# BillyXYB/TransEditor

Hardware: AMD Instinct MI355X
Metric: 256x256 images/sec/GPU, G+D fwd+bwd, batch 16; 1/2/4/8-GPU scaling (higher is better)
Workload: dtype f32

## Files before the change

include/te_hip.h:

```cpp
#ifndef TE_HIP_H
#define TE_HIP_H

#include <stdint.h>

#ifdef __cplusplus
extern "C" {
#endif

#define TE_ABI_VERSION 3

#define TE_ERR_NULL -1
#define TE_ERR_SHAPE -2
#define TE_ERR_UNSUPPORTED -3
#define TE_ERR_WORKSPACE -4

typedef void* te_stream_t;

int te_version(void);
const char* te_last_error_string(void);
const char* te_arch(void);

int te_bias_act_f32(float* out, const float* x, const float* b, const float* ref, int act, int grad,
                    float alpha, float scale, int64_t size_x, int64_t step_b, int64_t size_b,
                    te_stream_t stream);
// ... 20 lines not shown
                     int minor, int kh, int kw, int up_x, int up_y, int down_x, int down_y, int pad_x0,
                     int pad_x1, int pad_y0, int pad_y1, te_stream_t stream);
int te_upfirdn2d_f64(double* out, const double* x, const double* k, int64_t major, int in_h, int in_w,
                     int minor, int kh, int kw, int up_x, int up_y, int down_x, int down_y, int pad_x0,
                     int pad_x1, int pad_y0, int pad_y1, te_stream_t stream);


#define TE_CONV_3X3 0
#define TE_CONV_T2 1
#define TE_CONV_S2 2
#define TE_CONV_1X1 3
#define TE_CONV_3X3W 4
#define TE_CONV_3X3W6 5

#define TE_CONV_S2S6 6

#define TE_CONV_T2S6 7

#define TE_CONV_1X1S6 8

#define TE_PACK_FWD 0
#define TE_PACK_DGRAD 1
#define TE_PACK_SWAP 2
#define TE_PACK_WFWD 3
#define TE_PACK_WDGRAD 4
#define TE_PACK_W6FWD 5
#define TE_PACK_W6DGRAD 6
#define TE_PACK_S6FWD 7
#define TE_PACK_S6SWAP 8
#define TE_PACK_T6FWD 9
#define TE_PACK_T6SWAP 10
#define TE_PACK_P6FWD 11
#define TE_PACK_P6DGRAD 12

int64_t te_conv_packed_numel(int kind_pack, int Co, int Ci, int ksize);
int te_conv_pack_weights_f32(float* wp, const float* w, float wscale, int kind_pack, int Co, int Ci,
                             int ksize, te_stream_t stream);
int te_conv_pack_weights2_f32(float* wp_a, int kind_a, float* wp_b, int kind_b, const float* w, float wscale, int Co, int Ci,
                              int ksize, te_stream_t stream);

int te_conv_pack_weights_multi_f32(int n, float* const* wp, const float* const* w, const float* wscale, const int* kind_pack,
                                   const int* Co, const int* Ci, const int* ksize, te_stream_t stream);

int te_conv_f32(float* out, const float* in, const float* wp, const float* isc, const float* osc,
                const float* bias, int act, int kind, int B, int K, int M, int H, int W,
                te_stream_t stream);
int te_conv_splitk_count(int kind, int B, int K, int M, int H, int W);
int te_conv_wino_supported(int B, int K, int M, int H, int W);
int te_conv_wino6_supported(int B, int K, int M, int H, int W);
int te_conv_s2s6_supported(int B, int K, int M, int H, int W);
int te_conv_t2s6_supported(int B, int K, int M, int H, int W);
int te_conv_p1s6_supported(int B, int K, int M, int H, int W);
int te_conv_wino6_form(int form);
int te_conv_s2s6_form(int form);
int te_conv_t2s6_form(int form);
int64_t te_conv_t2s6_ws_floats(int B, int K, int H);
int te_conv_ws_f32(float* out, float* ws, const float* in, const float* wp, const float* isc, const float* osc,
                   const float* bias, int act, int kind, int B, int K, int M, int H, int W, te_stream_t stream);
int te_conv_res_f32(float* out, float* ws, const float* in, const float* wp, const float* isc, const float* osc,
                    const float* bias, const float* res, const float* mask_ref, float mask_gain, int act, int kind, int B,
                    int K, int M, int H, int W, te_stream_t stream);

int te_wgrad_slab_count(int kind, int B, int Co, int Ci, int H, int W);
int te_wgrad_pair_form(int kind, int Co, int Ci, int H, int W);
int te_wgrad_split_supported(int kind, int Co, int Ci, int H, int W);
int te_wgrad_split_bf16(int on);
int te_wgrad_t2_wide(int on);
enum { TE_WG6_FP32 = 0, TE_WG6_3X3 = 1, TE_WG6_3X3_PAIR = 2, TE_WG6_T2_WIDE = 3, TE_WG6_T2 = 4, TE_WG6_T2_MASKED = 5, TE_WG6_1X1 = 6 };
int te_wgrad6_form(int kind, int B, int Co, int Ci, int H, int W, int NB);
int te_wgrad_f32(float* slabs, const float* g, const float* x, int kind, int B, int Co, int Ci, int H,
                 int W, int S, te_stream_t stream);
int te_wgrad_group_plan(int kind, int B, int Co, int Ci, int H, int W, int* NB, int* S);
int te_wgrad_group_f32(float* slabs, const float* g, const float* x, int kind, int B, int Co, int Ci, int H, int W, int S, int NB,
                       te_stream_t stream);

int64_t te_wgrad_reduce_ws_floats(int B, int S, int Co, int Ci, int taps, int want_w, int want_isc, int want_osc);
int te_wgrad_reduce_f32(float* gw, float* gisc, float* gosc, float* ws, const float* slabs, const float* w,
                        float wscale, const float* isc, const float* osc, int B, int S, int Co, int Ci,
                        int taps, te_stream_t stream);

int te_rgb_supported(int M, int K, int HW);
int te_rgb_fwd_f32(float* out, const float* x, const float* w, const float* isc, const float* bias, float wscale, int B,
                   int K, int HW, te_stream_t stream);
int te_rgb_dgrad_f32(float* gx, const float* g, const float* w, const float* isc, float wscale, int B, int K, int HW,
                     te_stream_t stream);
int te_rgb_expand_f32(float* out, const float* x3, const float* w, const float* bias, int act, float wscale, int B, int K,
                      int HW, te_stream_t stream);
int te_rgb_wgrad_slab_count(int B, int K, int HW);
int te_rgb_wgrad_f32(float* slabs, const float* g, const float* x, int B, int K, int HW, int S, te_stream_t stream);
int te_rgb_wgrad_sum_f32(float* slabs, const float* g, const float* x, int B, int K, int HW, int S, te_stream_t stream);

int te_attn_fwd_f32(float* o, float* sim, const float* q, const float* k, const float* v, float scale,
                    int N, int G, int M, int L, int D, te_stream_t stream);
int te_attn_bwd_f32(float* gq, float* gk, float* gv, const float* go, const float* gsim_or_null,
                    const float* q, const float* k, const float* v, const float* sim, float scale, int N,
                    int G, int M, int L, int D, te_stream_t stream);

int te_blur_actgrad_tiles(int in_h, int in_w, int kh, int kw, int pad_x0, int pad_x1, int pad_y0, int pad_y1);
int te_blur_actgrad_f32(float* gx, float* partial, const float* g, const float* ref, const float* k, int64_t major, int in_h,
                        int in_w, int kh, int kw, int pad_x0, int pad_x1, int pad_y0, int pad_y1, float alpha, float scale,
                        te_stream_t stream);
int te_blur_gradact_f32(float* gx, float* partial, const float* g, const float* ref, const float* k, int64_t major, int in_h,
                        int in_w, int kh, int kw, int pad_x0, int pad_x1, int pad_y0, int pad_y1, float alpha, float scale,
                        te_stream_t stream);

int te_small_gemm_f32(float* c, float* pre, const float* a, const float* b, const float* bias, const float* residual,
// ... 90 lines not shown
```

transeditor_amd/_lib.py:

```python
import ctypes as C
import os

import torch

_HERE = os.path.dirname(os.path.abspath(__file__))
LIB_PATH = os.path.join(_HERE, 'libte_hip.so')
_lib = None

CONV_3X3, CONV_T2, CONV_S2, CONV_1X1, CONV_3X3W, CONV_3X3W6, CONV_S2S6, CONV_T2S6, CONV_1X1S6 = 0, 1, 2, 3, 4, 5, 6, 7, 8
(PACK_FWD, PACK_DGRAD, PACK_SWAP, PACK_WFWD, PACK_WDGRAD, PACK_W6FWD, PACK_W6DGRAD, PACK_S6FWD, PACK_S6SWAP, PACK_T6FWD,
 PACK_T6SWAP, PACK_P6FWD, PACK_P6DGRAD) = range(13)

_P, _I, _L, _F = C.c_void_p, C.c_int, C.c_int64, C.c_float
_SIGNATURES = {
    'te_version': (C.c_int, []),
    'te_last_error_string': (C.c_char_p, []),
    'te_arch': (C.c_char_p, []),
    'te_bias_act_f32': (C.c_int, [_P, _P, _P, _P, _I, _I, _F, _F, _L, _L, _L, _P]),
    'te_bias_act_f16': (C.c_int, [_P, _P, _P, _P, _I, _I, _F, _F, _L, _L, _L, _P]),
    'te_bias_act_f64': (C.c_int, [_P, _P, _P, _P, _I, _I, _F, _F, _L, _L, _L, _P]),
    'te_bias_act_bwd_ws_floats': (C.c_int64, [_L, _L, _L]),
    'te_bias_act_bwd_f32': (C.c_int, [_P, _P, _P, _P, _P, _F, _F, _L, _L, _L, _P]),
    'te_bias_act_bwd_rgb_supported': (C.c_int, [_L, _L, _L]),
    'te_bias_act_bwd_rgb_f32': (C.c_int, [_P, _P, _P, _P, _P, _P, _P, _P, _F, _F, _F, _L, _L, _L, _P]),
    'te_upfirdn2d_f32': (C.c_int, [_P, _P, _P, _L, _I, _I, _I, _I, _I, _I, _I, _I, _I, _I, _I, _I, _I,
                                   _P, _L, _I, _F, _F, _P]),
    'te_upfirdn2d_f16': (C.c_int, [_P, _P, _P, _L, _I, _I, _I, _I, _I, _I, _I, _I, _I, _I, _I, _I, _I, _P]),
    'te_upfirdn2d_f64': (C.c_int, [_P, _P, _P, _L, _I, _I, _I, _I, _I, _I, _I, _I, _I, _I, _I, _I, _I, _P]),
    'te_conv_packed_numel': (C.c_int64, [_I, _I, _I, _I]),
    'te_conv_pack_weights_f32': (C.c_int, [_P, _P, _F, _I, _I, _I, _I, _P]),
    'te_conv_pack_weights2_f32': (C.c_int, [_P, _I, _P, _I, _P, _F, _I, _I, _I, _P]),
    'te_conv_pack_weights_multi_f32': (C.c_int, [_I, _P, _P, _P, _P, _P, _P, _P, _P]),
    'te_conv_f32': (C.c_int, [_P, _P, _P, _P, _P, _P, _I, _I, _I, _I, _I, _I, _I, _P]),
    'te_conv_splitk_count': (C.c_int, [_I, _I, _I, _I, _I, _I]),
    'te_conv_wino_supported': (C.c_int, [_I, _I, _I, _I, _I]),
    'te_conv_wino6_supported': (C.c_int, [_I, _I, _I, _I, _I]),
    'te_conv_wino6_form': (C.c_int, [_I]),
    'te_conv_s2s6_form': (C.c_int, [_I]),
    'te_conv_t2s6_form': (C.c_int, [_I]),
    'te_conv_t2s6_ws_floats': (C.c_int64, [_I, _I, _I]),
    'te_conv_s2s6_supported': (C.c_int, [_I, _I, _I, _I, _I]),
    'te_conv_t2s6_supported': (C.c_int, [_I, _I, _I, _I, _I]),
    'te_conv_p1s6_supported': (C.c_int, [_I, _I, _I, _I, _I]),
    'te_conv_ws_f32': (C.c_int, [_P, _P, _P, _P, _P, _P, _P, _I, _I, _I, _I, _I, _I, _I, _P]),
    'te_conv_res_f32': (C.c_int, [_P, _P, _P, _P, _P, _P, _P, _P, _P, _F, _I, _I, _I, _I, _I, _I, _I, _P]),
    'te_wgrad_slab_count': (C.c_int, [_I, _I, _I, _I, _I, _I]),
    'te_wgrad_pair_form': (C.c_int, [_I, _I, _I, _I, _I]),
    'te_wgrad_split_supported': (C.c_int, [_I, _I, _I, _I, _I]),
    'te_wgrad_split_bf16': (C.c_int, [_I]),
    'te_wgrad_t2_wide': (C.c_int, [_I]),
    'te_wgrad6_form': (C.c_int, [_I, _I, _I, _I, _I, _I, _I]),
    'te_wgrad_f32': (C.c_int, [_P, _P, _P, _I, _I, _I, _I, _I, _I, _I, _P]),
    'te_wgrad_group_plan': (C.c_int, [_I, _I, _I, _I, _I, _I, _P, _P]),
    'te_wgrad_group_f32': (C.c_int, [_P, _P, _P, _I, _I, _I, _I, _I, _I, _I, _I, _P]),
    'te_wgrad_reduce_ws_floats': (C.c_int64, [_I, _I, _I, _I, _I, _I, _I, _I]),
    'te_wgrad_reduce_f32': (C.c_int, [_P, _P, _P, _P, _P, _P, _F, _P, _P, _I, _I, _I, _I, _I, _P]),
    'te_rgb_supported': (C.c_int, [_I, _I, _I]),
    'te_rgb_fwd_f32': (C.c_int, [_P, _P, _P, _P, _P, _F, _I, _I, _I, _P]),
    'te_rgb_dgrad_f32': (C.c_int, [_P, _P, _P, _P, _F, _I, _I, _I, _P]),
    'te_rgb_wgrad_sum_f32': (C.c_int, [_P, _P, _P, _I, _I, _I, _I, _P]),
    'te_rgb_expand_f32': (C.c_int, [_P, _P, _P, _P, _I, _F, _I, _I, _I, _P]),
    'te_rgb_wgrad_slab_count': (C.c_int, [_I, _I, _I]),
    'te_rgb_wgrad_f32': (C.c_int, [_P, _P, _P, _I, _I, _I, _I, _P]),
    'te_blur_actgrad_tiles': (C.c_int, [_I] * 8),
    'te_blur_actgrad_f32': (C.c_int, [_P, _P, _P, _P, _P, _L, _I, _I, _I, _I, _I, _I, _I, _I, _F, _F, _P]),
    'te_blur_gradact_f32': (C.c_int, [_P, _P, _P, _P, _P, _L, _I, _I, _I, _I, _I, _I, _I, _I, _F, _F, _P]),
    'te_small_gemm_f32': (C.c_int, [_P, _P, _P, _P, _P, _P, _P, _F, _I, _I, _I, _L, _L, _L, _L, _F, _F, _I, _P]),
    'te_small_gemm_batched_f32': (C.c_int, [_P, _P, _P, _P, _I, _L, _L, _L, _L, _P, _P, _I, _I, _I, _L, _L, _L, _L, _L, _L,
                                             _F, _F, _I, _P]),
    'te_layer_norm_supported': (C.c_int, [_L, _I]),
    'te_layer_norm_fwd_f32': (C.c_int, [_P, _P, _P, _L, _I, _F, _P]),
    'te_layer_norm_bwd_f32': (C.c_int, [_P, _P, _P, _P, _L, _I, _P]),
    'te_pixel_norm_supported': (C.c_int, [_L, _I, _I]),
    'te_pixel_norm_fwd_f32': (C.c_int, [_P, _P, _P, _L, _I, _I, _F, _P]),
    'te_pixel_norm_bwd_f32': (C.c_int, [_P, _P, _P, _P, _L, _I, _I, _P]),
    'te_demod_fwd_f32': (C.c_int, [_P, _P, _P, _P, _F, _F, _I, _I, _I, _I, _P]),
    'te_demod_bwd_f32': (C.c_int, [_P, _P, _P, _P, _P, _P, _P, _F, _I, _I, _I, _I, _I, _P]),
    'te_attn_fwd_f32': (C.c_int, [_P, _P, _P, _P, _P, _F, _I, _I, _I, _I, _I, _P]),
    'te_attn_bwd_f32': (C.c_int, [_P, _P, _P, _P, _P, _P, _P, _P, _P, _F, _I, _I, _I, _I, _I, _P]),
    'te_small_gemm_splitk_f32': (C.c_int, [_P, _P, _P, _I, _P, _P, _P, _P, _I, _I, _I, _L, _L, _L, _L, _F, _F, _I, _P]),
    'te_minibatch_stddev_fwd_f32': (C.c_int, [_P, _P, _I, _I, _I, _I, _F, _P]),
    'te_minibatch_stddev_bwd_f32': (C.c_int, [_P, _P, _P, _I, _I, _I, _I, _F, _P]),
    'te_mt_adam_f32': (C.c_int, [_P, _P, _I, _I, _I, C.c_double, C.c_double, C.c_double, C.c_double, _I, _P]),
    'te_mt_ema_f32': (C.c_int, [_P, _P, _I, _I, _I, C.c_double, _P]),
    'te_chan_scale_f32': (C.c_int, [_P, _P, _P, _L, _L, _P]),
    'te_chan_dot_f32': (C.c_int, [_P, _P, _P, _L, _L, _P]),
    'te_lpips_stem_fwd_f32': (C.c_int, [_P, _P, _P, _P, _I, _I, _I, _P]),
    'te_lpips_stem_dgrad_f32': (C.c_int, [_P, _P, _P, _P, _I, _I, _I, _P]),
    'te_maxpool2_fwd_f32': (C.c_int, [_P, _P, _L, _I, _I, _P]),
    'te_maxpool2_bwd_f32': (C.c_int, [_P, _P, _P, _L, _I, _I, _P]),
# ... 226 lines not shown
    Co, Ci, ks, _ = w.shape
    n = lib().te_conv_packed_numel(kind_pack, Co, Ci, ks)
    wp = torch.empty(n, device=w.device, dtype=w.dtype)
    _check(lib().te_conv_pack_weights_f32(_ptr(wp), _ptr(w), wscale, kind_pack, Co, Ci, ks, _stream()),
           'te_conv_pack_weights_f32')
    return wp


def conv_pack2(w, kind_a, kind_b, wscale=1.0):
    w = w.contiguous()
    Co, Ci, ks, _ = w.shape
    wa = torch.empty(lib().te_conv_packed_numel(kind_a, Co, Ci, ks), device=w.device, dtype=w.dtype)
    wb = torch.empty(lib().te_conv_packed_numel(kind_b, Co, Ci, ks), device=w.device, dtype=w.dtype)
    _check(lib().te_conv_pack_weights2_f32(_ptr(wa), kind_a, _ptr(wb), kind_b, _ptr(w), wscale, Co, Ci, ks, _stream()),
           'te_conv_pack_weights2_f32')
    return wa, wb


def conv_pack_multi(jobs):
    n = len(jobs)
    if not n:
        return
    for wp, w, _, _ in jobs:
        if not (w.is_contiguous() and wp.is_contiguous()):
            raise RuntimeError('te_hip: conv_pack_multi needs dense weights and buffers')
    arr = lambda ty, vals: (ty * n)(*vals)
    _check(lib().te_conv_pack_weights_multi_f32(
        n, arr(C.c_void_p, [_ptr(j[0]) for j in jobs]), arr(C.c_void_p, [_ptr(j[1]) for j in jobs]),
        arr(C.c_float, [float(j[3]) for j in jobs]), arr(C.c_int, [int(j[2]) for j in jobs]),
        arr(C.c_int, [j[1].shape[0] for j in jobs]), arr(C.c_int, [j[1].shape[1] for j in jobs]),
        arr(C.c_int, [j[1].shape[2] for j in jobs]), _stream()), 'te_conv_pack_weights_multi_f32')


def wino_ok(B, K, M, H, W):
    return bool(lib().te_conv_wino_supported(B, K, M, H, W))


def s2s6_ok(B, K, M, H, W):
    return bool(lib().te_conv_s2s6_supported(B, K, M, H, W))


def t2s6_ok(B, K, M, H, W):
    return bool(lib().te_conv_t2s6_supported(B, K, M, H, W))


def p1s6_ok(B, K, M, H, W):
    return bool(lib().te_conv_p1s6_supported(B, K, M, H, W))


def wino6_form(form=-1):
    return int(lib().te_conv_wino6_form(form))


def s2s6_form(form=-1):
    return int(lib().te_conv_s2s6_form(form))


def t2s6_form(form=-1):
    return int(lib().te_conv_t2s6_form(form))


def wino6_ok(B, K, M, H, W):
    return bool(lib().te_conv_wino6_supported(B, K, M, H, W))


def conv_out_shape(kind, B, M, H, W):
    if kind in (CONV_T2, CONV_T2S6):
        return (B, M, 2 * H + 1, 2 * W + 1)
    return (B, M, H, W)


def _aligned16(t):
    if t is None or t.data_ptr() % 16 == 0:
        return t
    return t.clone(memory_format=torch.contiguous_format)


def conv(x, wp, kind, M, H, W, isc=None, osc=None, bias=None, act=0, res=None, mask_ref=None, mask_gain=1.0):
    x = x.contiguous()
    if kind == CONV_1X1S6:
        x = _aligned16(x)
    res = _aligned16(res.contiguous()) if res is not None else None
    mask_ref = _aligned16(mask_ref.contiguous()) if mask_ref is not None else None
    B, K = x.shape[0], x.shape[1]
    out = torch.empty(conv_out_shape(kind, B, M, H, W), device=x.device, dtype=x.dtype)
    if res is not None and tuple(res.shape) != tuple(out.shape):
        raise RuntimeError(f'te_hip: residual {tuple(res.shape)} does not match the convolution output {tuple(out.shape)}')
    if mask_ref is not None and tuple(mask_ref.shape) != tuple(out.shape):
        raise RuntimeError(f'te_hip: mask reference {tuple(mask_ref.shape)} does not match the convolution output {tuple(out.shape)}')
    S = lib().te_conv_splitk_count(kind, B, K, M, H, W)
    if S < 1:
        raise RuntimeError(f'te_conv_splitk_count failed ({S})')
    ws = torch.empty((S,) + tuple(out.shape), device=x.device, dtype=x.dtype) if S > 1 else None
    if kind == CONV_T2S6:
        ws = torch.empty(B * K * H, device=x.device, dtype=x.dtype)
    _check(lib().te_conv_res_f32(_ptr(out), _ptr(ws), _ptr(x), _ptr(wp), _ptr(isc), _ptr(osc), _ptr(bias),
                                 _ptr(res), _ptr(mask_ref), mask_gain, act, kind, B, K, M, H, W,
                                 _stream()),
           'te_conv_res_f32')
    return out


def wgrad_slabs(g, x, kind, H, W, group=False):
    g, x = g.contiguous(), x.contiguous()
    B, Co, Ci = g.shape[0], g.shape[1], x.shape[1]
    taps = 1 if kind == CONV_1X1 else 9
# ... 636 lines not shown
```

transeditor_amd/csrc/split6_common.h:

```cpp
#pragma once
#include "conv_common.h"

typedef short bf16x8 __attribute__((ext_vector_type(8)));
typedef __bf16 bf16x2 __attribute__((ext_vector_type(2)));
typedef float f32x2 __attribute__((ext_vector_type(2)));
typedef float f32x2u __attribute__((ext_vector_type(2), aligned(4)));
typedef float f32x4u __attribute__((ext_vector_type(4), aligned(4)));
typedef unsigned u32x4 __attribute__((ext_vector_type(4)));

__device__ __forceinline__ void split6_barrier() { asm volatile("s_waitcnt lgkmcnt(0)\n\ts_barrier" ::: "memory"); }
__device__ __forceinline__ void split6_wait_vm() { asm volatile("s_waitcnt vmcnt(0)" ::: "memory"); }

__device__ __forceinline__ unsigned split6_piece(float te, float to) {
    const f32x2 t = {te, to};
    return __builtin_bit_cast(unsigned, __builtin_convertvector(t, bf16x2));
}
__device__ __forceinline__ unsigned split6_take(float te, float to, float& fe, float& fo) {
    const unsigned h = split6_piece(te, to);
    fe = __builtin_bit_cast(float, h << 16);
    fo = __builtin_bit_cast(float, h & 0xFFFF0000u);
    return h;
}
__device__ __forceinline__ void split6_pin(float& te, float& to, float& fe, float& fo) { asm volatile("" : "+v"(te), "+v"(to), "+v"(fe), "+v"(fo)); }
template <bool PIN_LOW = true>
__device__ __forceinline__ void split6_step4(int j, float ve, float vo, float& te, float& to, float& fe, float& fo, unsigned& h, unsigned& m, unsigned& l) {
    if (j == 0) {
        te = ve; to = vo;
        h = split6_take(te, to, fe, fo);
    } else if (j == 1) {
        te -= fe; to -= fo;
    } else if (j == 2) {
        m = split6_take(te, to, fe, fo);
    } else {
        te -= fe; to -= fo;
        l = split6_piece(te, to);
        if (PIN_LOW) asm volatile("" : "+v"(l));
    }
    split6_pin(te, to, fe, fo);
}
__device__ __forceinline__ void split6_step3(int j, float ve, float vo, float& te, float& to, float& fe, float& fo, unsigned& h, unsigned& m, unsigned& l) {
    if (j == 0) {
        te = ve; to = vo;
        h = split6_take(te, to, fe, fo);
    } else if (j == 1) {
        te -= fe; to -= fo;
        m = split6_take(te, to, fe, fo);
    } else {
        te -= fe; to -= fo;
        l = split6_piece(te, to);
    }
    split6_pin(te, to, fe, fo);
}

__device__ __forceinline__ void split6_product(int q, const bf16x8 (&a)[3], const bf16x8 (&b)[3], f32x16& big, f32x16& small) {
    constexpr int PA[6] = {1, 0, 2, 0, 1, 0}, PB[6] = {1, 2, 0, 1, 0, 0};
    f32x16& d = q < 5 ? small : big;
    d = __builtin_amdgcn_mfma_f32_32x32x16_bf16(a[PA[q]], b[PB[q]], d, 0, 0, 0);
}

__device__ __forceinline__ bool split6_tile(int ntiles, int nt8, int mblocks, int& tile, int& mb) {
    const int xcd = blockIdx.x & 7, jx = blockIdx.x >> 3;
    const int tq = jx / mblocks;
    mb = jx % mblocks;
    tile = nt8 ? (int)(((int64_t)xcd * ntiles) >> 3) + tq : tq * 8 + xcd;
    return tile < (nt8 ? (int)(((int64_t)(xcd + 1) * ntiles) >> 3) : ntiles);
}

template <auto KERNEL, class Args>
inline void split6_launch(dim3 grid, int threads, size_t lds, hipStream_t s, const Args& a) {
    static std::atomic<uint64_t> attr_done{0};
    te::allow_big_lds(attr_done, (const void*)KERNEL, 160 * 1024);
    KERNEL<<<grid, threads, lds, s>>>(a);
}
#define SPLIT6_LAUNCH_ISC(kernel, isc, blocks, threads, lds, s, a) \
    ((isc) ? split6_launch<kernel<true>>(blocks, threads, lds, s, a) : split6_launch<kernel<false>>(blocks, threads, lds, s, a))
```

transeditor_amd/csrc/wino6.hip:

```cpp
#include "split6_common.h"
#ifdef W6P_PROF
#define TE_PROF
#endif
#include "te_prof.h"

namespace {

constexpr int WT = 512, KC = 16, TW = 32, NP = TW / 2, BM = 64, TH = 8;
constexpr int U_CHUNKS = 36 * 2 * 64;

struct Wino6Args {
    float* out; const float* in; const u32x4* U; const float* isc; const float* osc; const float* bias; const float* res;
    const float* mref; float mgain; int act;
    int B, K, M, H, W, ntiles, mblocks, tiles_x, tiles_y, nt8;
    int lgpw;
};

constexpr int PH = 4, PR = PH + 2;
constexpr int TP_PLANE = PR * 2 * NP * 4;
constexpr int TP_DWORDS = 12 * TP_PLANE;
constexpr int GT = WT / 2;
constexpr int P_IN = (PR * NP * 8) / GT;
static_assert(PR * NP * 8 == P_IN * GT, "items must divide over the group");

PROF_BUFFER(w6p, 2048 * 8 * 8)
constexpr int SLOT0 = 21;

template <bool ISC>
__global__ __launch_bounds__(WT, 2) void wino6p_kernel(const Wino6Args p) {
    extern __shared__ __attribute__((aligned(16))) unsigned char smem_raw[];
    u32x4* ul = reinterpret_cast<u32x4*>(smem_raw);
    const int tid = threadIdx.x, lane = tid & 63, l31 = lane & 31, half = lane >> 5;
    const int wid = __builtin_amdgcn_readfirstlane(tid >> 6);
    const int grp = wid >> 2, wq = wid & 3, wm = wq >> 1, wrl = wq & 1, gt = tid & (GT - 1);
    unsigned* tl = reinterpret_cast<unsigned*>(smem_raw + U_CHUNKS * 16) + grp * TP_DWORDS;
    const u32x4* tl4 = reinterpret_cast<const u32x4*>(tl);
    int tile, mb;
    if (!split6_tile(p.ntiles, p.nt8, p.mblocks, tile, mb)) return;
    const int pwm = (1 << p.lgpw) - 1;
    const int tx = tile % p.tiles_x, ty = (tile / p.tiles_x) % p.tiles_y, b = (tile / (p.tiles_x * p.tiles_y)) << (4 - p.lgpw);
    const int x0 = tx * TW, y0 = ty * TH, yh = y0 + PH * grp;
    const float* inb = p.in + (size_t)b * p.K * p.H * p.W;
    const float* iscb = ISC ? p.isc + (size_t)b * p.K : nullptr;
    const bool has_left = x0 == 0, has_right = x0 + TW >= p.W, has_rowout = (yh == 0) || (yh + PH == p.H);

    f32x16 acc[4];
#pragma unroll
    for (int c = 0; c < 4; ++c)
#pragma unroll
        for (int r = 0; r < 16; ++r) acc[c][r] = 0.f;

    unsigned g_off[P_IN];
    int l_off[P_IN], e_flag[P_IN];
#pragma unroll
    for (int i = 0; i < P_IN; ++i) {
        const int e = gt + GT * i;
        const int jj = e & 15, q = (e >> 4) & 7, row = e >> 7;
        const int gy = yh - 1 + row;
        const int sj = jj >> p.lgpw, jl = jj & pwm;
        const bool left = x0 == 0 && jl == 0, right = x0 + TW >= p.W && jl == pwm, rowout = gy < 0 || gy >= p.H;
        e_flag[i] = (left ? 1 : 0) | (right ? 2 : 0) | (rowout ? 4 : 0);
        const int gyc = gy < 0 ? 0 : (gy >= p.H ? p.H - 1 : gy);
        g_off[i] = (unsigned)(sj * p.K * p.H * p.W + (2 * q * p.H + gyc) * p.W + x0 + 2 * jl - 1 + (left ? 1 : 0) - (right ? 1 : 0));
        l_off[i] = ((row * 2 + (q >> 2)) * NP + jj) * 4 + (q & 3);
    }
    const unsigned q2 = 2u * ((gt >> 4) & 7) + (unsigned)(((gt & 15) >> p.lgpw) * p.K);
    const size_t plane = (size_t)p.H * p.W;
// ... 159 lines not shown
    const size_t off0 = ((size_t)bo * p.M + mbase) * plane + (size_t)(y0 + 2 * wr + rr) * p.W + x0 + 2 * (jj & pwm);
    const float g_pos = p.act == 3 ? 1.4142135623730951f : 1.f;
    float scv[16], biv[16];
#pragma unroll
    for (int r = 0; r < 16; ++r) {
        const int m = mbase + (r & 3) + 8 * (r >> 2) + 4 * half;
        scv[r] = p.osc ? p.osc[(size_t)bo * p.M + m] : 1.f;
        biv[r] = p.bias ? p.bias[m] : 0.f;
    }
    f32x2 resv[16], mrefv[16];
    if (p.res) {
#pragma unroll
        for (int r = 0; r < 16; ++r)
            resv[r] = *reinterpret_cast<const f32x2*>(p.res + off0 + (size_t)((r & 3) + 8 * (r >> 2) + 4 * half) * plane);
    }
    if (p.mref) {
#pragma unroll
        for (int r = 0; r < 16; ++r)
            mrefv[r] = *reinterpret_cast<const f32x2*>(p.mref + off0 + (size_t)((r & 3) + 8 * (r >> 2) + 4 * half) * plane);
    }
#pragma unroll
    for (int r = 0; r < 16; ++r) {
        const int dm = (r & 3) + 8 * (r >> 2) + 4 * half;
        float v0 = acc[0][r] + acc[1][r] + acc[2][r];
        float v1 = acc[1][r] - acc[2][r] - acc[3][r];
        const float sc = scv[r], bi = biv[r];
        v0 = v0 * sc + bi;
        v1 = v1 * sc + bi;
        if (p.act >= 3) {
            v0 = (v0 > 0.f ? v0 : v0 * 0.2f) * g_pos;
            v1 = (v1 > 0.f ? v1 : v1 * 0.2f) * g_pos;
        }
        const size_t o = off0 + (size_t)dm * plane;
        if (p.res) { v0 += resv[r][0]; v1 += resv[r][1]; }
        if (p.mref) {
            v0 *= mrefv[r][0] > 0.f ? p.mgain : 0.2f * p.mgain;
            v1 *= mrefv[r][1] > 0.f ? p.mgain : 0.2f * p.mgain;
        }
        f32x2 v; v[0] = v0; v[1] = v1;
        *reinterpret_cast<f32x2*>(p.out + o) = v;
    }
}


template <bool ISC>
__global__ __launch_bounds__(WT, 2) void wino6q_kernel(const Wino6Args p) {
    extern __shared__ __attribute__((aligned(16))) unsigned char smem_raw[];
    u32x4* ul = reinterpret_cast<u32x4*>(smem_raw);
    const int tid = threadIdx.x, lane = tid & 63, l31 = lane & 31, half = lane >> 5;
    const int wid = __builtin_amdgcn_readfirstlane(tid >> 6);
    const int grp = wid >> 2, wq = wid & 3, wm = wq >> 1, wrl = wq & 1, gt = tid & (GT - 1);
    unsigned* tl = reinterpret_cast<unsigned*>(smem_raw + U_CHUNKS * 16) + grp * TP_DWORDS;
    const u32x4* tl4 = reinterpret_cast<const u32x4*>(tl);
    int tile, mbq;
    if (!split6_tile(p.ntiles, p.nt8, p.mblocks, tile, mbq)) return;
    const int tx = tile % p.tiles_x, ty = (tile / p.tiles_x) % p.tiles_y, b = tile / (p.tiles_x * p.tiles_y);
    const int x0 = tx * TW, y0 = ty * TH, yh = y0 + PH * grp;
    const float* inb = p.in + (size_t)b * p.K * p.H * p.W;
    const float* iscb = ISC ? p.isc + (size_t)b * p.K : nullptr;
    const bool has_left = x0 == 0, has_right = x0 + TW == p.W, has_rowout = (yh == 0) || (yh + PH == p.H);

    f32x16 acc[2][4];
#pragma unroll
    for (int m = 0; m < 2; ++m)
#pragma unroll
        for (int c = 0; c < 4; ++c)
#pragma unroll
            for (int r = 0; r < 16; ++r) acc[m][c][r] = 0.f;

    unsigned g_off[P_IN];
    int l_off[P_IN], e_flag[P_IN];
#pragma unroll
    for (int i = 0; i < P_IN; ++i) {
        const int e = gt + GT * i;
        const int jj = e & 15, q = (e >> 4) & 7, row = e >> 7;
        const int gy = yh - 1 + row;
        const bool left = x0 == 0 && jj == 0, right = x0 + TW == p.W && jj == NP - 1, rowout = gy < 0 || gy >= p.H;
        e_flag[i] = (left ? 1 : 0) | (right ? 2 : 0) | (rowout ? 4 : 0);
        const int gyc = gy < 0 ? 0 : (gy >= p.H ? p.H - 1 : gy);
        g_off[i] = (unsigned)((2 * q * p.H + gyc) * p.W + x0 + 2 * jj - 1 + (left ? 1 : 0) - (right ? 1 : 0));
        l_off[i] = ((row * 2 + (q >> 2)) * NP + jj) * 4 + (q & 3);
    }
    const unsigned q2 = 2u * ((gt >> 4) & 7);
    const size_t plane = (size_t)p.H * p.W;
    const int MT = p.M >> 5;
    f32x4 rin[P_IN][2];
    f32x2 rsc = {1.f, 1.f};
    const int nstage = p.K / KC, nimg = 2 * nstage;
    auto fetch_scales = [&](int s) {
        if (ISC) rsc = *reinterpret_cast<const f32x2u*>(iscb + s * KC + q2);
    };
    auto fetch_item = [&](int i, int s) {
#pragma unroll
        for (int h2 = 0; h2 < 2; ++h2)
            rin[i][h2] = *reinterpret_cast<const f32x4u*>(inb + ((size_t)s * KC + h2) * plane + g_off[i]);
    };
    auto issue_u = [&](int uh, int j) {
        const u32x4* us = p.U + (size_t)(j >> 1) * 36 * MT * 64;
        const int mb = 2 * mbq + (j & 1);
#pragma unroll
        for (int r = 0; r < 9; ++r) {
            const int jw = wq * 9 + r, piece = jw / 12, rem = jw % 12, kc = (rem >> 1) + 6 * uh, mt = rem & 1;
            const int pk = piece * 12 + kc;
            const u32x4* g = us + ((size_t)pk * MT + 2 * mb + mt) * 64 + (unsigned)lane;
            __builtin_amdgcn_global_load_lds((const __attribute__((address_space(1))) void*)g,
                                             (__attribute__((address_space(3))) void*)(ul + (pk * 2 + mt) * 64), 16, 0, 0);
        }
    };
    unsigned res[P_IN][4][3];
    float te = 0.f, to = 0.f, fe = 0.f, fo = 0.f;
    constexpr int N_SLOT = 3 + 4 * 4 * P_IN;
    auto arith = [&](int k) {
        if (k < 0) {
        } else if (k < P_IN) {
#pragma unroll
            for (int h2 = 0; h2 < 2; ++h2) {
                f32x4 v = rin[k][h2];
                if (has_left) {
                    int f = e_flag[k];
                    asm volatile("" : "+v"(f) :: "memory");
                    if (f & 1) { v[3] = v[2]; v[2] = v[1]; v[1] = v[0]; v[0] = 0.f; }
                }
                if (has_right) {
                    int f = e_flag[k];
                    asm volatile("" : "+v"(f) :: "memory");
                    if (f & 2) { v[0] = v[1]; v[1] = v[2]; v[2] = v[3]; v[3] = 0.f; }
                }
                if (has_rowout) {
                    int f = e_flag[k];
                    asm volatile("" : "+v"(f) :: "memory");
                    if (f & 4) { v[0] = 0.f; v[1] = 0.f; v[2] = 0.f; v[3] = 0.f; }
                }
                rin[k][h2] = ISC ? v * rsc[h2] : v;
                asm volatile("" : "+v"(rin[k][h2]));
            }
        } else if (k < N_SLOT) {
            const int u = (k - P_IN) >> 2, j = (k - P_IN) & 3, i = u >> 2, c = u & 3;
            float ve = 0.f, vo = 0.f;
            if (j == 0) {
                const f32x4 e = rin[i][0], o = rin[i][1];
                ve = c == 0 ? e[0] - e[2] : (c == 1 ? e[1] + e[2] : (c == 2 ? e[2] - e[1] : e[1] - e[3]));
                vo = c == 0 ? o[0] - o[2] : (c == 1 ? o[1] + o[2] : (c == 2 ? o[2] - o[1] : o[1] - o[3]));
            }
            split6_step4(j, ve, vo, te, to, fe, fo, res[i][c][0], res[i][c][1], res[i][c][2]);
        }
    };
    auto write_res = [&]() {
#pragma unroll
        for (int i = 0; i < P_IN; ++i)
#pragma unroll
            for (int c = 0; c < 4; ++c)
#pragma unroll
                for (int pc = 0; pc < 3; ++pc) tl[l_off[i] + (pc * 4 + c) * TP_PLANE] = res[i][c][pc];
    };
    const int rr = l31 >> 4, jj = l31 & 15;
    const int b_chunk = ((2 * wrl + rr) * 2 + half) * NP + jj;
    const int a_chunk = wm * 64 + lane;

    auto multiply = [&](auto mset_tag, int fs) {
        constexpr int MSET = decltype(mset_tag)::value;
        bf16x8 av[2][3], bv[2][3];
        auto rd1 = [&](int g, int slot, int q) {
            const int ky = g >> 2, c = g & 3;
            if (q < 3) av[slot][q] = __builtin_bit_cast(bf16x8, ul[a_chunk + ((q * 3 + ky) * 4 + c) * 128]);
            else bv[slot][q - 3] = __builtin_bit_cast(bf16x8, tl4[b_chunk + (((q - 3) * 4 + c) * PR + ky) * 2 * NP]);
        };
#pragma unroll
        for (int q = 0; q < 6; ++q) rd1(0, 0, q);
        __builtin_amdgcn_s_setprio(1);
#pragma unroll
        for (int g = 0; g < 12; ++g) {
            const int slot = g & 1, c = g & 3;
            if (g == 5) split6_barrier();
            __builtin_amdgcn_sched_barrier(0);
#pragma unroll
            for (int q = 0; q < 6; ++q) {
                split6_product(q, av[slot], bv[slot], acc[MSET][c], acc[MSET][c]);
                if (g + 1 < 12 && q < 3) { rd1(g + 1, slot ^ 1, 2 * q); rd1(g + 1, slot ^ 1, 2 * q + 1); }
                const int k = g * 6 + q;
                if (MSET == 0) {
                    if (k == 5) fetch_scales(fs);
#pragma unroll
                    for (int i = 0; i < P_IN; ++i)
                        if (k == 6 + 12 * i) fetch_item(i, fs);
                } else {
                    arith(k - SLOT0);
                }
                __builtin_amdgcn_sched_barrier(0);
            }
        }
        __builtin_amdgcn_s_setprio(0);
        split6_barrier();
    };
    auto stage = [&](int ph, bool write) {
        const int cs = (ph + 1) >> 1;
        const bool work = cs >= 1 && cs < nimg;
        if (grp == 1 && work) issue_u(1, cs);
        __builtin_amdgcn_sched_barrier(0);
        if (write) write_res();
        if (grp == 1 && work) split6_wait_vm();
        split6_barrier();
        if (grp == 0 && work) {
            issue_u(0, cs);
            split6_wait_vm();
        }
        split6_barrier();
    };

    fetch_scales(0);
#pragma unroll
    for (int i = 0; i < P_IN; ++i) fetch_item(i, 0);
    if (grp == 0) { issue_u(0, 0); issue_u(1, 0); }
#pragma unroll
    for (int k = 0; k < N_SLOT; ++k) arith(k);
    write_res();
    split6_wait_vm();
    split6_barrier();
    int ph = 0;
    if (grp == 1) { stage(0, false); ph = 1; }
    for (int s = 0; s < nstage; ++s) {
        const int fs = min(s + 1, nstage - 1);
        multiply(std::integral_constant<int, 0>{}, fs);
        stage(ph + 1, false);
        multiply(std::integral_constant<int, 1>{}, fs);
        if (!(grp == 1 && s == nstage - 1)) stage(ph + 3, true);
        ph += 4;
    }

    const int wr = grp * 2 + wrl;
    const float g_pos = p.act == 3 ? 1.4142135623730951f : 1.f;
#pragma unroll
    for (int m = 0; m < 2; ++m) {
        const int mbase = (2 * mbq + m) * BM + wm * 32;
        const size_t off0 = ((size_t)b * p.M + mbase) * plane + (size_t)(y0 + 2 * wr + rr) * p.W + x0 + 2 * jj;
        float scv[16], biv[16];
#pragma unroll
        for (int r = 0; r < 16; ++r) {
            const int mm = mbase + (r & 3) + 8 * (r >> 2) + 4 * half;
            scv[r] = p.osc ? p.osc[(size_t)b * p.M + mm] : 1.f;
            biv[r] = p.bias ? p.bias[mm] : 0.f;
        }
        f32x2 resv[16], mrefv[16];
        if (p.res) {
#pragma unroll
            for (int r = 0; r < 16; ++r)
                resv[r] = *reinterpret_cast<const f32x2*>(p.res + off0 + (size_t)((r & 3) + 8 * (r >> 2) + 4 * half) * plane);
        }
        if (p.mref) {
#pragma unroll
            for (int r = 0; r < 16; ++r)
                mrefv[r] = *reinterpret_cast<const f32x2*>(p.mref + off0 + (size_t)((r & 3) + 8 * (r >> 2) + 4 * half) * plane);
        }
#pragma unroll
        for (int r = 0; r < 16; ++r) {
            const int dm = (r & 3) + 8 * (r >> 2) + 4 * half;
            float v0 = acc[m][0][r] + acc[m][1][r] + acc[m][2][r];
            float v1 = acc[m][1][r] - acc[m][2][r] - acc[m][3][r];
            const float sc = scv[r], bi = biv[r];
            v0 = v0 * sc + bi;
            v1 = v1 * sc + bi;
            if (p.act >= 3) {
                v0 = (v0 > 0.f ? v0 : v0 * 0.2f) * g_pos;
                v1 = (v1 > 0.f ? v1 : v1 * 0.2f) * g_pos;
            }
            const size_t o = off0 + (size_t)dm * plane;
            if (p.res) { v0 += resv[r][0]; v1 += resv[r][1]; }
            if (p.mref) {
                v0 *= mrefv[r][0] > 0.f ? p.mgain : 0.2f * p.mgain;
                v1 *= mrefv[r][1] > 0.f ? p.mgain : 0.2f * p.mgain;
            }
            f32x2 v; v[0] = v0; v[1] = v1;
            *reinterpret_cast<f32x2*>(p.out + o) = v;
        }
    }
}

}

static std::atomic<int> g_w6_form{2};
extern "C" int te_conv_wino6_form(int form) {
    const int old = g_w6_form.load(std::memory_order_relaxed);
    if (form >= 1 && form <= 3) g_w6_form.store(form, std::memory_order_relaxed);
    return old;
}

PROF_READBACK(w6p)

extern "C" int te_conv_wino6_supported(int B, int K, int M, int H, int W) {
    if (!(B > 0 && K >= 32 && K % 32 == 0 && M >= BM && M % BM == 0 && H >= TH && H % TH == 0)) return 0;
    const bool wide = W >= TW && W % TW == 0, pair16 = W == 16 && B % 2 == 0;
    if (!wide && !pair16) return 0;
    const int64_t tiles = wide ? (int64_t)B * (H / TH) * (W / TW) : (int64_t)(B / 2) * (H / TH);
    if (!wide && tiles * (M / BM) < te::kNumCU / 2) return 0;
    return ((int64_t)K * H * W * 4 * (wide ? 1 : 2) < 0x7FFFFFFF && tiles * (M / BM) < 0x7FFFFFF0) ? 1 : 0;
}

int te_wino6_launch(float* out, const float* in, const float* U, const float* isc, const float* osc, const float* bias, const float* res,
                    const float* mask_ref, float mask_gain, int act, int B, int K, int M, int H, int W, hipStream_t s) {
    TE_REQUIRE(te_conv_wino6_supported(B, K, M, H, W), TE_ERR_UNSUPPORTED,
               "te_conv_f32(TE_CONV_3X3W6): needs K %% 32 == 0, M %% 64 == 0, W %% 32 == 0 (or W == 16 and an even batch), H %% 8 == 0 (te_conv_wino6_supported)");
    TE_REQUIRE(((reinterpret_cast<uintptr_t>(out) | reinterpret_cast<uintptr_t>(U) | reinterpret_cast<uintptr_t>(res) |
                 reinterpret_cast<uintptr_t>(mask_ref)) & 15) == 0 && (reinterpret_cast<uintptr_t>(in) & 3) == 0, TE_ERR_UNSUPPORTED,
               "te_conv_f32(TE_CONV_3X3W6): 16-byte aligned tensors required");
    Wino6Args a{};
    a.out = out; a.in = in; a.U = reinterpret_cast<const u32x4*>(U); a.isc = isc; a.osc = osc; a.bias = bias; a.res = res;
    a.mref = mask_ref; a.mgain = mask_gain; a.act = act;
    a.B = B; a.K = K; a.M = M; a.H = H; a.W = W;
    a.lgpw = W >= TW ? 4 : 3;
    a.tiles_x = W >= TW ? W / TW : 1; a.tiles_y = H / TH; a.mblocks = M / BM;
    a.ntiles = (W >= TW ? B : B / 2) * a.tiles_x * a.tiles_y;
    a.nt8 = te::xcd_banded() ? (int)te::cdiv(a.ntiles, 8) : 0;
    const int64_t blocks = te::cdiv(a.ntiles, 8) * 8 * a.mblocks;
    const int form = g_w6_form.load(std::memory_order_relaxed);
    const int64_t blocks_q = te::cdiv(a.ntiles, 8) * 8 * (M / (2 * BM));
    if (form >= 2 && M % (2 * BM) == 0 && W >= TW && (form == 3 || blocks_q >= te::kNumCU)) {
        a.mblocks = M / (2 * BM);
        const int64_t blocks2 = blocks_q;
        const size_t lds = (size_t)U_CHUNKS * 16 + 2 * (size_t)TP_DWORDS * 4;
        SPLIT6_LAUNCH_ISC(wino6q_kernel, isc, dim3((unsigned)blocks2), WT, lds, s, a);
    } else {
        const size_t lds = (size_t)U_CHUNKS * 16 + 2 * (size_t)TP_DWORDS * 4;
        SPLIT6_LAUNCH_ISC(wino6p_kernel, isc, dim3((unsigned)blocks), WT, lds, s, a);
    }
    return te::launch_status("te_conv_f32(TE_CONV_3X3W6)");
}
```

Measured before the change: 151.5.

## Make wino6q kernel persistent over tile lists, prefetching the next tile's data

```diff
diff --git a/include/te_hip.h b/include/te_hip.h
--- a/include/te_hip.h
+++ b/include/te_hip.h
@@ -96,6 +96,7 @@
 int te_conv_t2s6_supported(int B, int K, int M, int H, int W);
 int te_conv_p1s6_supported(int B, int K, int M, int H, int W);
 int te_conv_wino6_form(int form);
+int te_conv_wino6_tiles_per_block(int n);
 int te_conv_s2s6_form(int form);
 int te_conv_t2s6_form(int form);
 int64_t te_conv_t2s6_ws_floats(int B, int K, int H);
diff --git a/transeditor_amd/_lib.py b/transeditor_amd/_lib.py
--- a/transeditor_amd/_lib.py
+++ b/transeditor_amd/_lib.py
@@ -36,6 +36,7 @@
     'te_conv_wino_supported': (C.c_int, [_I, _I, _I, _I, _I]),
     'te_conv_wino6_supported': (C.c_int, [_I, _I, _I, _I, _I]),
     'te_conv_wino6_form': (C.c_int, [_I]),
+    'te_conv_wino6_tiles_per_block': (C.c_int, [_I]),
     'te_conv_s2s6_form': (C.c_int, [_I]),
     'te_conv_t2s6_form': (C.c_int, [_I]),
     'te_conv_t2s6_ws_floats': (C.c_int64, [_I, _I, _I]),
@@ -368,6 +369,10 @@
     return int(lib().te_conv_wino6_form(form))
 
 
+def wino6_tiles_per_block(n=-1):
+    return int(lib().te_conv_wino6_tiles_per_block(n))
+
+
 def s2s6_form(form=-1):
     return int(lib().te_conv_s2s6_form(form))
 
diff --git a/transeditor_amd/csrc/split6_common.h b/transeditor_amd/csrc/split6_common.h
--- a/transeditor_amd/csrc/split6_common.h
+++ b/transeditor_amd/csrc/split6_common.h
@@ -66,6 +66,24 @@
     return tile < (nt8 ? (int)(((int64_t)(xcd + 1) * ntiles) >> 3) : ntiles);
 }
 
+__device__ __forceinline__ bool split6_tile_list(int ntiles, int nt8, int mblocks, int lists, int& tile, int& end, int& step, int& mb) {
+    step = nt8 ? 1 : 8;
+    if (lists == 0) {
+        const bool has = split6_tile(ntiles, nt8, mblocks, tile, mb);
+        end = tile + step;
+        return has;
+    }
+    const int xcd = blockIdx.x & 7, jx = blockIdx.x >> 3;
+    const int lq = jx / mblocks;
+    mb = jx % mblocks;
+    const int first = nt8 ? (int)(((int64_t)xcd * ntiles) >> 3) : xcd;
+    const int nb = nt8 ? (int)(((int64_t)(xcd + 1) * ntiles) >> 3) - first : (ntiles - xcd + 7) >> 3;
+    const int lo = (int)((int64_t)lq * nb / lists), hi = (int)((int64_t)(lq + 1) * nb / lists);
+    tile = first + step * lo;
+    end = first + step * hi;
+    return lo < hi;
+}
+
 template <auto KERNEL, class Args>
 inline void split6_launch(dim3 grid, int threads, size_t lds, hipStream_t s, const Args& a) {
     static std::atomic<uint64_t> attr_done{0};
diff --git a/transeditor_amd/csrc/wino6.hip b/transeditor_amd/csrc/wino6.hip
--- a/transeditor_amd/csrc/wino6.hip
+++ b/transeditor_amd/csrc/wino6.hip
@@ -1,4 +1,5 @@
 #include "split6_common.h"
+#include "wino6_schedule.h"
 #ifdef W6P_PROF
 #define TE_PROF
 #endif
@@ -13,6 +14,7 @@
     float* out; const float* in; const u32x4* U; const float* isc; const float* osc; const float* bias; const float* res;
     const float* mref; float mgain; int act;
     int B, K, M, H, W, ntiles, mblocks, tiles_x, tiles_y, nt8;
+    int lists;
     int lgpw;
 };
 
@@ -278,13 +280,11 @@
     const int grp = wid >> 2, wq = wid & 3, wm = wq >> 1, wrl = wq & 1, gt = tid & (GT - 1);
     unsigned* tl = reinterpret_cast<unsigned*>(smem_raw + U_CHUNKS * 16) + grp * TP_DWORDS;
     const u32x4* tl4 = reinterpret_cast<const u32x4*>(tl);
-    int tile, mbq;
-    if (!split6_tile(p.ntiles, p.nt8, p.mblocks, tile, mbq)) return;
-    const int tx = tile % p.tiles_x, ty = (tile / p.tiles_x) % p.tiles_y, b = tile / (p.tiles_x * p.tiles_y);
-    const int x0 = tx * TW, y0 = ty * TH, yh = y0 + PH * grp;
-    const float* inb = p.in + (size_t)b * p.K * p.H * p.W;
-    const float* iscb = ISC ? p.isc + (size_t)b * p.K : nullptr;
-    const bool has_left = x0 == 0, has_right = x0 + TW == p.W, has_rowout = (yh == 0) || (yh + PH == p.H);
+    int tile, tile_end, tile_step, mbq;
+    if (!split6_tile_list(p.ntiles, p.nt8, p.mblocks, p.lists, tile, tile_end, tile_step, mbq)) return;
+    const float* inb;
+    const float* iscb = nullptr;
+    bool has_left, has_right, has_rowout;
 
     f32x16 acc[2][4];
 #pragma unroll
@@ -296,15 +296,38 @@
 
     unsigned g_off[P_IN];
     int l_off[P_IN], e_flag[P_IN];
+    typedef const __attribute__((address_space(4))) Wino6Args* KArgs;
+    auto kargs = [&]() {
+        KArgs k = (KArgs)__builtin_amdgcn_kernarg_segment_ptr();
+        asm volatile("" : "+s"(k));
+        return k;
+    };
+    auto set_tile = [&](int t) {
+        const KArgs a = kargs();
+        const int aH = a->H, aW = a->W, atx = a->tiles_x, aty = a->tiles_y, aK = a->K;
+        const int tx = t % atx, ty = (t / atx) % aty, b = t / (atx * aty);
+        const int x0 = tx * TW, yh = ty * TH + PH * grp;
+        inb = a->in + (size_t)b * aK * aH * aW;
+        if (ISC) iscb = a->isc + (size_t)b * aK;
+        has_left = x0 == 0; has_right = x0 + TW == aW; has_rowout = (yh == 0) || (yh + PH == aH);
+        int gto = gt;
+        asm volatile("" : "+v"(gto));
+#pragma unroll
+        for (int i = 0; i < P_IN; ++i) {
+            const int e = gto + GT * i;
+            const int jj = e & 15, q = (e >> 4) & 7, row = e >> 7;
+            const int gy = yh - 1 + row;
+            const bool left = x0 == 0 && jj == 0, right = x0 + TW == aW && jj == NP - 1, rowout = gy < 0 || gy >= aH;
+            e_flag[i] = (left ? 1 : 0) | (right ? 2 : 0) | (rowout ? 4 : 0);
+            const int gyc = gy < 0 ? 0 : (gy >= aH ? aH - 1 : gy);
+            g_off[i] = (unsigned)((2 * q * aH + gyc) * aW + x0 + 2 * jj - 1 + (left ? 1 : 0) - (right ? 1 : 0));
+        }
+    };
+    set_tile(tile);
 #pragma unroll
     for (int i = 0; i < P_IN; ++i) {
         const int e = gt + GT * i;
         const int jj = e & 15, q = (e >> 4) & 7, row = e >> 7;
-        const int gy = yh - 1 + row;
-        const bool left = x0 == 0 && jj == 0, right = x0 + TW == p.W && jj == NP - 1, rowout = gy < 0 || gy >= p.H;
-        e_flag[i] = (left ? 1 : 0) | (right ? 2 : 0) | (rowout ? 4 : 0);
-        const int gyc = gy < 0 ? 0 : (gy >= p.H ? p.H - 1 : gy);
-        g_off[i] = (unsigned)((2 * q * p.H + gyc) * p.W + x0 + 2 * jj - 1 + (left ? 1 : 0) - (right ? 1 : 0));
         l_off[i] = ((row * 2 + (q >> 2)) * NP + jj) * 4 + (q & 3);
     }
     const unsigned q2 = 2u * ((gt >> 4) & 7);
@@ -322,15 +345,21 @@
             rin[i][h2] = *reinterpret_cast<const f32x4u*>(inb + ((size_t)s * KC + h2) * plane + g_off[i]);
     };
     auto issue_u = [&](int uh, int j) {
-        const u32x4* us = p.U + (size_t)(j >> 1) * 36 * MT * 64;
-        const int mb = 2 * mbq + (j & 1);
-#pragma unroll
-        for (int r = 0; r < 9; ++r) {
-            const int jw = wq * 9 + r, piece = jw / 12, rem = jw % 12, kc = (rem >> 1) + 6 * uh, mt = rem & 1;
-            const int pk = piece * 12 + kc;
-            const u32x4* g = us + ((size_t)pk * MT + 2 * mb + mt) * 64 + (unsigned)lane;
-            __builtin_amdgcn_global_load_lds((const __attribute__((address_space(1))) void*)g,
-                                             (__attribute__((address_space(3))) void*)(ul + (pk * 2 + mt) * 64), 16, 0, 0);
+        int wqo = wq;
+        asm volatile("" : "+s"(wqo));
+        const u32x4* us = p.U + ((size_t)(j >> 1) * 36 * MT + 2 * (2 * mbq + (j & 1))) * 64;
+        const unsigned pstride = 12u * (unsigned)MT * 64u;
+#pragma unroll
+        for (int t = 0; t < 3; ++t) {
+            const int rem = wqo * 3 + t, kc = (rem >> 1) + 6 * uh, mt = rem & 1;
+            const u32x4* g0 = us + (unsigned)(kc * MT + mt) * 64u;
+            u32x4* l0 = ul + (kc * 2 + mt) * 64;
+#pragma unroll
+            for (int piece = 0; piece < 3; ++piece) {
+                const u32x4* g = g0 + piece * pstride + (unsigned)lane;
+                __builtin_amdgcn_global_load_lds((const __attribute__((address_space(1))) void*)g,
+                                                 (__attribute__((address_space(3))) void*)(l0 + piece * 24 * 64), 16, 0, 0);
+            }
         }
     };
     unsigned res[P_IN][4][3];
@@ -418,16 +447,17 @@
         __builtin_amdgcn_s_setprio(0);
         split6_barrier();
     };
-    auto stage = [&](int ph, bool write) {
-        const int cs = (ph + 1) >> 1;
-        const bool work = cs >= 1 && cs < nimg;
-        if (grp == 1 && work) issue_u(1, cs);
+    auto stage = [&](int ph, bool write, bool has_next) {
+        const int cs = wino6_sched::renew_image(ph);
+        const bool work = wino6_sched::renew_work(cs, nimg, has_next);
+        const int ci = cs == nimg ? 0 : cs;
+        if (grp == 1 && work) issue_u(1, ci);
         __builtin_amdgcn_sched_barrier(0);
         if (write) write_res();
         if (grp == 1 && work) split6_wait_vm();
         split6_barrier();
         if (grp == 0 && work) {
-            issue_u(0, cs);
+            issue_u(0, ci);
             split6_wait_vm();
         }
         split6_barrier();
@@ -442,62 +472,89 @@
     write_res();
     split6_wait_vm();
     split6_barrier();
-    int ph = 0;
-    if (grp == 1) { stage(0, false); ph = 1; }
-    for (int s = 0; s < nstage; ++s) {
-        const int fs = min(s + 1, nstage - 1);
-        multiply(std::integral_constant<int, 0>{}, fs);
-        stage(ph + 1, false);
-        multiply(std::integral_constant<int, 1>{}, fs);
-        if (!(grp == 1 && s == nstage - 1)) stage(ph + 3, true);
-        ph += 4;
-    }
-
-    const int wr = grp * 2 + wrl;
-    const float g_pos = p.act == 3 ? 1.4142135623730951f : 1.f;
-#pragma unroll
-    for (int m = 0; m < 2; ++m) {
-        const int mbase = (2 * mbq + m) * BM + wm * 32;
-        const size_t off0 = ((size_t)b * p.M + mbase) * plane + (size_t)(y0 + 2 * wr + rr) * p.W + x0 + 2 * jj;
-        float scv[16], biv[16];
-#pragma unroll
-        for (int r = 0; r < 16; ++r) {
-            const int mm = mbase + (r & 3) + 8 * (r >> 2) + 4 * half;
-            scv[r] = p.osc ? p.osc[(size_t)b * p.M + mm] : 1.f;
-            biv[r] = p.bias ? p.bias[mm] : 0.f;
-        }
-        f32x2 resv[16], mrefv[16];
-        if (p.res) {
-#pragma unroll
-            for (int r = 0; r < 16; ++r)
-                resv[r] = *reinterpret_cast<const f32x2*>(p.res + off0 + (size_t)((r & 3) + 8 * (r >> 2) + 4 * half) * plane);
-        }
-        if (p.mref) {
-#pragma unroll
-            for (int r = 0; r < 16; ++r)
-                mrefv[r] = *reinterpret_cast<const f32x2*>(p.mref + off0 + (size_t)((r & 3) + 8 * (r >> 2) + 4 * half) * plane);
-        }
-#pragma unroll
-        for (int r = 0; r < 16; ++r) {
-            const int dm = (r & 3) + 8 * (r >> 2) + 4 * half;
-            float v0 = acc[m][0][r] + acc[m][1][r] + acc[m][2][r];
-            float v1 = acc[m][1][r] - acc[m][2][r] - acc[m][3][r];
-            const float sc = scv[r], bi = biv[r];
-            v0 = v0 * sc + bi;
-            v1 = v1 * sc + bi;
-            if (p.act >= 3) {
-                v0 = (v0 > 0.f ? v0 : v0 * 0.2f) * g_pos;
-                v1 = (v1 > 0.f ? v1 : v1 * 0.2f) * g_pos;
-            }
-            const size_t o = off0 + (size_t)dm * plane;
-            if (p.res) { v0 += resv[r][0]; v1 += resv[r][1]; }
-            if (p.mref) {
-                v0 *= mrefv[r][0] > 0.f ? p.mgain : 0.2f * p.mgain;
-                v1 *= mrefv[r][1] > 0.f ? p.mgain : 0.2f * p.mgain;
-            }
-            f32x2 v; v[0] = v0; v[1] = v1;
-            *reinterpret_cast<f32x2*>(p.out + o) = v;
-        }
+    for (;;) {
+        const bool has_next = tile + tile_step < tile_end;
+        int ph = 0;
+        if (wino6_sched::lead_phase(grp)) { stage(0, false, has_next); ph = 1; }
+        for (int s = 0; s < nstage; ++s) {
+            bool next_tile;
+            const int fs = wino6_sched::fetch_stage(s, nstage, has_next, next_tile);
+            if (next_tile) set_tile(tile + tile_step);
+            multiply(std::integral_constant<int, 0>{}, fs);
+            stage(ph + 1, false, has_next);
+            multiply(std::integral_constant<int, 1>{}, fs);
+            if (wino6_sched::runs_sb(grp, s, nstage, has_next)) stage(ph + 3, true, has_next);
+            ph += 4;
+        }
+        for (int i = 0; i < wino6_sched::tail_barriers(grp, has_next); ++i) split6_barrier();
+
+        const KArgs e = kargs();
+        const int tx = tile % e->tiles_x, ty = (tile / e->tiles_x) % e->tiles_y, b = tile / (e->tiles_x * e->tiles_y);
+        const int x0 = tx * TW, y0 = ty * TH;
+        int elane = lane;
+        asm volatile("" : "+v"(elane));
+        const int ehalf = elane >> 5, err = (elane & 31) >> 4, ejj = elane & 15;
+        const int wr = grp * 2 + wrl;
+        const int eM = e->M, eW = e->W, eact = e->act;
+        const size_t eplane = (size_t)e->H * eW;
+        const float emgain = e->mgain;
+        const float g_pos = eact == 3 ? 1.4142135623730951f : 1.f;
+        float* const eout = e->out;
+        const float* const eosc = e->osc; const float* const ebias = e->bias; const float* const eres = e->res; const float* const emref = e->mref;
+#pragma unroll
+        for (int m = 0; m < 2; ++m) {
+            const int mbase = (2 * mbq + m) * BM + wm * 32;
+            const size_t off0 = ((size_t)b * eM + mbase) * eplane + (size_t)(y0 + 2 * wr) * eW + x0;
+            const unsigned lo = (unsigned)(err * eW + 2 * ejj) + 4u * (unsigned)ehalf * (unsigned)eplane;
+#pragma unroll
+            for (int r0 = 0; r0 < 16; r0 += 4) {
+                float scv[4], biv[4];
+#pragma unroll
+                for (int r = r0; r < r0 + 4; ++r) {
+                    const int mm = mbase + (r & 3) + 8 * (r >> 2) + 4 * ehalf;
+                    scv[r - r0] = eosc ? eosc[(size_t)b * eM + mm] : 1.f;
+                    biv[r - r0] = ebias ? ebias[mm] : 0.f;
+                }
+                f32x2 resv[4], mrefv[4];
+                if (eres) {
+#pragma unroll
+                    for (int r = r0; r < r0 + 4; ++r)
+                        resv[r - r0] = *reinterpret_cast<const f32x2*>(eres + off0 + (size_t)((r & 3) + 8 * (r >> 2)) * eplane + lo);
+                }
+                if (emref) {
+#pragma unroll
+                    for (int r = r0; r < r0 + 4; ++r)
+                        mrefv[r - r0] = *reinterpret_cast<const f32x2*>(emref + off0 + (size_t)((r & 3) + 8 * (r >> 2)) * eplane + lo);
+                }
+#pragma unroll
+                for (int r = r0; r < r0 + 4; ++r) {
+                    float v0 = acc[m][0][r] + acc[m][1][r] + acc[m][2][r];
+                    float v1 = acc[m][1][r] - acc[m][2][r] - acc[m][3][r];
+                    const float sc = scv[r - r0], bi = biv[r - r0];
+                    v0 = v0 * sc + bi;
+                    v1 = v1 * sc + bi;
+                    if (eact >= 3) {
+                        v0 = (v0 > 0.f ? v0 : v0 * 0.2f) * g_pos;
+                        v1 = (v1 > 0.f ? v1 : v1 * 0.2f) * g_pos;
+                    }
+                    if (eres) { v0 += resv[r - r0][0]; v1 += resv[r - r0][1]; }
+                    if (emref) {
+                        v0 *= mrefv[r - r0][0] > 0.f ? emgain : 0.2f * emgain;
+                        v1 *= mrefv[r - r0][1] > 0.f ? emgain : 0.2f * emgain;
+                    }
+                    f32x2 v; v[0] = v0; v[1] = v1;
+                    *reinterpret_cast<f32x2*>(eout + off0 + (size_t)((r & 3) + 8 * (r >> 2)) * eplane + lo) = v;
+                }
+            }
+        }
+        if (!has_next) break;
+        tile += tile_step;
+#pragma unroll
+        for (int m = 0; m < 2; ++m)
+#pragma unroll
+            for (int c = 0; c < 4; ++c)
+#pragma unroll
+                for (int r = 0; r < 16; ++r) acc[m][c][r] = 0.f;
     }
 }
 
@@ -508,6 +565,23 @@
     const int old = g_w6_form.load(std::memory_order_relaxed);
     if (form >= 1 && form <= 3) g_w6_form.store(form, std::memory_order_relaxed);
     return old;
+}
+
+constexpr int W6_MAX_TPB = 4096;
+static std::atomic<int> g_w6_tpb{0};
+extern "C" int te_conv_wino6_tiles_per_block(int n) {
+    const int old = g_w6_tpb.load(std::memory_order_relaxed);
+    if (n >= 0 && n <= W6_MAX_TPB) g_w6_tpb.store(n, std::memory_order_relaxed);
+    return old;
+}
+
+static int w6_auto_tpb(int nt8c, int mblocks) {
+    const int64_t rounds1 = te::cdiv((int64_t)8 * nt8c * mblocks, te::kNumCU);
+    for (int n = 4; n >= 2; --n) {
+        const int64_t blocks = (int64_t)8 * te::cdiv(nt8c, n) * mblocks;
+        if (blocks >= te::kNumCU && te::cdiv(blocks, te::kNumCU) * n <= rounds1) return n;
+    }
+    return 1;
 }
 
 PROF_READBACK(w6p)
@@ -541,7 +615,11 @@
     const int64_t blocks_q = te::cdiv(a.ntiles, 8) * 8 * (M / (2 * BM));
     if (form >= 2 && M % (2 * BM) == 0 && W >= TW && (form == 3 || blocks_q >= te::kNumCU)) {
         a.mblocks = M / (2 * BM);
-        const int64_t blocks2 = blocks_q;
+        const int nt8c = (int)te::cdiv(a.ntiles, 8);
+        int tpb = g_w6_tpb.load(std::memory_order_relaxed);
+        if (tpb == 0) tpb = w6_auto_tpb(nt8c, a.mblocks);
+        a.lists = tpb >= 2 ? (int)te::cdiv(nt8c, tpb) : 0;
+        const int64_t blocks2 = a.lists ? (int64_t)8 * a.lists * a.mblocks : blocks_q;
         const size_t lds = (size_t)U_CHUNKS * 16 + 2 * (size_t)TP_DWORDS * 4;
         SPLIT6_LAUNCH_ISC(wino6q_kernel, isc, dim3((unsigned)blocks2), WT, lds, s, a);
     } else {
diff --git a/transeditor_amd/csrc/wino6_schedule.h b/transeditor_amd/csrc/wino6_schedule.h
--- /dev/null
+++ b/transeditor_amd/csrc/wino6_schedule.h
@@ -0,0 +1,70 @@
+#pragma once
+
+#if defined(__HIPCC__) || defined(__CUDACC__)
+#define W6S_HD __host__ __device__ __forceinline__
+#else
+#define W6S_HD inline
+#endif
+
+namespace wino6_sched {
+
+W6S_HD constexpr bool lead_phase(int grp) { return grp == 1; }
+W6S_HD constexpr int renew_image(int ph) { return (ph + 1) >> 1; }
+W6S_HD constexpr bool renew_work(int cs, int nimg, bool has_next) { return cs >= 1 && (cs < nimg || has_next); }
+W6S_HD constexpr int fetch_stage(int s, int nstage, bool has_next, bool& next_tile) {
+    next_tile = s == nstage - 1 && has_next;
+    return s + 1 < nstage ? s + 1 : (has_next ? 0 : s);
+}
+W6S_HD constexpr bool runs_sb(int grp, int s, int nstage, bool has_next) { return !(grp == 1 && s == nstage - 1) || has_next; }
+W6S_HD constexpr int tail_barriers(int grp, bool has_next) { return grp == 0 && has_next ? 2 : 0; }
+
+#if !defined(__HIP_DEVICE_COMPILE__)
+enum Kind { BARRIER, READ_UA, READ_UB, DMA_UA, DMA_UB, DMA_WAIT, READ_T, WRITE_T, EPILOGUE };
+struct Event { int kind, tile, idx; };
+
+template <class F>
+void replay(int grp, int nstage, int ntile, F&& emit) {
+    const int nimg = 2 * nstage;
+    auto ev = [&](int k, int t = 0, int i = 0) { emit(Event{k, t, i}); };
+    auto multiply = [&](int t, int s, int m) {
+        ev(READ_T, t, s); ev(READ_UA, t, 2 * s + m);
+        ev(BARRIER);
+        ev(READ_T, t, s); ev(READ_UB, t, 2 * s + m);
+        ev(BARRIER);
+    };
+    auto stage = [&](int t, int ph, bool has_next, bool write, int wt, int ws) {
+        const int cs = renew_image(ph);
+        const bool work = renew_work(cs, nimg, has_next);
+        const int it = cs == nimg ? t + 1 : t, ii = cs == nimg ? 0 : cs;
+        if (grp == 1 && work) ev(DMA_UB, it, ii);
+        if (write) ev(WRITE_T, wt, ws);
+        if (grp == 1 && work) ev(DMA_WAIT);
+        ev(BARRIER);
+        if (grp == 0 && work) { ev(DMA_UA, it, ii); ev(DMA_WAIT); }
+        ev(BARRIER);
+    };
+    if (grp == 0) { ev(DMA_UA, 0, 0); ev(DMA_UB, 0, 0); }
+    ev(WRITE_T, 0, 0);
+    ev(DMA_WAIT);
+    ev(BARRIER);
+    for (int t = 0; t < ntile; ++t) {
+        const bool has_next = t + 1 < ntile;
+        int ph = 0;
+        if (lead_phase(grp)) { stage(t, 0, has_next, false, 0, 0); ph = 1; }
+        for (int s = 0; s < nstage; ++s) {
+            bool next_tile = false;
+            const int fs = fetch_stage(s, nstage, has_next, next_tile);
+            const bool stale = fs == s;
+            multiply(t, s, 0);
+            stage(t, ph + 1, has_next, false, 0, 0);
+            multiply(t, s, 1);
+            if (runs_sb(grp, s, nstage, has_next)) stage(t, ph + 3, has_next, true, stale ? -1 : t + (next_tile ? 1 : 0), fs);
+            ph += 4;
+        }
+        for (int i = 0; i < tail_barriers(grp, has_next); ++i) ev(BARRIER);
+        ev(EPILOGUE, t);
+    }
+}
+#endif
+
+}
```

New measurement: 153.7, median of 6. 1.01x the previous value.
